# ganslate-team/ganslate

Measured on AMD Instinct MI355X. Metric: training images/sec, CycleGAN ResNet-9 256x256 bf16, higher is better.
Workload: dtype bf16; 1 GPU; horse2zebra CycleGAN ResNet-9 + PatchGAN-3, 256x256, batch 8 per GPU, lsgan, lambda 10/10, pool 50, Adam(2e-4, 0.5), SSIM + D-output metrics on; global_batch=8, parallelism=dp1

## Files before the change

### ganslate_amd/csrc/common.hpp

```cpp
#pragma once
#include <hip/hip_runtime.h>
#include <stdint.h>
#include <type_traits>
#include "../../include/ganslate_hip.h"

typedef __attribute__((ext_vector_type(8))) short bf16x8;
typedef __attribute__((ext_vector_type(4))) short s16x4;
typedef __attribute__((ext_vector_type(4))) float f32x4;
typedef __attribute__((ext_vector_type(2))) float f32x2;
typedef __attribute__((ext_vector_type(2))) __bf16 bf16x2_t;

#define GS_LDS(p) ((__attribute__((address_space(3))) void*)(p))
#define GS_GLB(p) ((const __attribute__((address_space(1))) void*)(p))

__device__ __forceinline__ float bf2f(unsigned short h) { return __uint_as_float(((unsigned)h) << 16); }
__device__ __forceinline__ float bf_lo(unsigned u) { return __uint_as_float(u << 16); }
__device__ __forceinline__ float bf_hi(unsigned u) { return __uint_as_float(u & 0xffff0000u); }
__device__ __forceinline__ unsigned pack_bf2(float a, float b) {
  f32x2 v = {a, b};
  bf16x2_t r = __builtin_convertvector(v, bf16x2_t);
  return *reinterpret_cast<unsigned*>(&r);
}
__device__ __forceinline__ unsigned short f2bf(float a) { return (unsigned short)(pack_bf2(a, 0.f) & 0xffffu); }
__device__ __forceinline__ void unpack_bf8(float* f, const uint4 v) {
  f[0] = bf_lo(v.x); f[1] = bf_hi(v.x); f[2] = bf_lo(v.y); f[3] = bf_hi(v.y);
  f[4] = bf_lo(v.z); f[5] = bf_hi(v.z); f[6] = bf_lo(v.w); f[7] = bf_hi(v.w);
}
__device__ __forceinline__ void add_bf8(float* f, const uint4 v) {
  f[0] += bf_lo(v.x); f[1] += bf_hi(v.x); f[2] += bf_lo(v.y); f[3] += bf_hi(v.y);
  f[4] += bf_lo(v.z); f[5] += bf_hi(v.z); f[6] += bf_lo(v.w); f[7] += bf_hi(v.w);
}
__device__ __forceinline__ uint4 pack_bf8(const float* f) {
  uint4 o;
  o.x = pack_bf2(f[0], f[1]); o.y = pack_bf2(f[2], f[3]); o.z = pack_bf2(f[4], f[5]); o.w = pack_bf2(f[6], f[7]);
  return o;
}

__device__ __forceinline__ void glds16(const void* gsrc, void* lds_wave_base) {
  __builtin_amdgcn_global_load_lds(GS_GLB(gsrc), GS_LDS(lds_wave_base), 16, 0, 0);
}

__device__ __forceinline__ unsigned lds_addr(const void* p) {
  return (unsigned)(size_t)(__attribute__((address_space(3))) const char*)p;
}
template <int OFF>
__device__ __forceinline__ void lds_read128(bf16x8& v, unsigned addr) {
  asm volatile("ds_read_b128 %0, %1 offset:%2" : "=v"(v) : "v"(addr), "i"(OFF) : "memory");
}
template <int N>
__device__ __forceinline__ void gs_lgkm_wait(bf16x8& a, bf16x8& b, bf16x8& c, bf16x8& d, bf16x8& e, bf16x8& f) {
  asm volatile("s_waitcnt lgkmcnt(%6)" : "+v"(a), "+v"(b), "+v"(c), "+v"(d), "+v"(e), "+v"(f) : "i"(N) : "memory");
}
template <int N>
__device__ __forceinline__ void gs_lgkm_wait(bf16x8& a, bf16x8& b, bf16x8& c, bf16x8& d, bf16x8& e) {
  asm volatile("s_waitcnt lgkmcnt(%5)" : "+v"(a), "+v"(b), "+v"(c), "+v"(d), "+v"(e) : "i"(N) : "memory");
}
template <int N>
__device__ __forceinline__ void gs_lgkm_wait(bf16x8& a, bf16x8& b, bf16x8& c, bf16x8& d, bf16x8& e, bf16x8& f,
                                             bf16x8& g, bf16x8& h) {
  asm volatile("s_waitcnt lgkmcnt(%8)"
               : "+v"(a), "+v"(b), "+v"(c), "+v"(d), "+v"(e), "+v"(f), "+v"(g), "+v"(h) : "i"(N) : "memory");
}

template <int N>
__device__ __forceinline__ void gs_lgkm_wait_only() { asm volatile("s_waitcnt lgkmcnt(%0)" ::"i"(N) : "memory"); }
__device__ __forceinline__ void reg_fence(bf16x8& x) { asm volatile("" : "+v"(x)); }

__device__ __forceinline__ void lds_barrier() {
  asm volatile("s_waitcnt lgkmcnt(0)" ::: "memory");
  __builtin_amdgcn_s_barrier();
  asm volatile("" ::: "memory");
}

template <int OFF>
__device__ __forceinline__ void lds_read64_tr(uint2& v, unsigned addr) {
  asm volatile("ds_read_b64_tr_b16 %0, %1 offset:%2" : "=v"(v) : "v"(addr), "i"(OFF) : "memory");
}
template <int N>
__device__ __forceinline__ void gs_lgkm_wait64(uint2& a, uint2& b) {
  asm volatile("s_waitcnt lgkmcnt(%2)" : "+v"(a), "+v"(b) : "i"(N) : "memory");
}
template <int N>
__device__ __forceinline__ void gs_lgkm_wait64(uint2& a, uint2& b, uint2& c, uint2& d, uint2& e, uint2& f) {
  asm volatile("s_waitcnt lgkmcnt(%6)" : "+v"(a), "+v"(b), "+v"(c), "+v"(d), "+v"(e), "+v"(f) : "i"(N) : "memory");
}
template <int B, int E, class F>
__device__ __forceinline__ void static_for(F&& f) {
  if constexpr (B < E) {
    f(std::integral_constant<int, B>{});
    static_for<B + 1, E>(f);
  }
}

__device__ __forceinline__ int div_small(int m, int d, float rcp) {
  int q = (int)((float)m * rcp);
  int r = m - q * d;
  if (r < 0) { --q; } else if (r >= d) { ++q; }
  return q;
}

__device__ __forceinline__ int border_index(int x, int n, int mode, bool& ok) {
  const bool inb = (unsigned)x < (unsigned)n;
  int xr = x < 0 ? -x : x;
  xr = xr >= n ? 2 * n - 2 - xr : xr;
  int xc = x < 0 ? 0 : x;
  xc = xc >= n ? n - 1 : xc;
  ok = ok & (inb | (mode != GS_BORDER_ZERO));
  return mode == GS_BORDER_REFLECT ? xr : (mode == GS_BORDER_REPLICATE ? xc : x);
}

__device__ __forceinline__ float apply_act(float v, int act, float slope) {
  if (act == GS_ACT_RELU) return v > 0.f ? v : 0.f;
  if (act == GS_ACT_LRELU) return v > 0.f ? v : v * slope;
  if (act == GS_ACT_TANH) return tanhf(v);
  return v;
}
static __device__ __noinline__ float gs_tanh_call(float v) { return tanhf(v); }
__device__ __forceinline__ float apply_act_small(float v, int act, float slope) {
  if (act == GS_ACT_RELU) return v > 0.f ? v : 0.f;
  if (act == GS_ACT_LRELU) return v > 0.f ? v : v * slope;
  if (act == GS_ACT_TANH) return gs_tanh_call(v);
  return v;
}
__device__ __forceinline__ float act_grad_from_out(float o, int act, float slope) {
  if (act == GS_ACT_RELU) return o > 0.f ? 1.f : 0.f;
  if (act == GS_ACT_LRELU) return o > 0.f ? 1.f : slope;
  if (act == GS_ACT_TANH) return 1.f - o * o;
  return 1.f;
}

__device__ __forceinline__ float inorm_dy(float g, float yh, float m, float s1, float s2, float rs) {
  const float gh = __fmul_rn(g, m);
  return __fmul_rn(rs, __fsub_rn(__fsub_rn(gh, s1), __fmul_rn(yh, s2)));
}

template <int CTRL>
__device__ __forceinline__ float dpp_mov(float v) {
  return __builtin_bit_cast(float, __builtin_amdgcn_update_dpp(0, __builtin_bit_cast(int, v), CTRL, 0xf, 0xf, false));
}
__device__ __forceinline__ float row16_sum(float v) {
  v += dpp_mov<0xB1>(v);
  v += dpp_mov<0x4E>(v);
  v += dpp_mov<0x141>(v);
  v += dpp_mov<0x140>(v);
  return v;
}
__device__ __forceinline__ float row_sum_stride4(float v) { v += dpp_mov<0x124>(v); v += dpp_mov<0x128>(v); return v; }
__device__ __forceinline__ float row_sum_stride8(float v) { v += dpp_mov<0x128>(v); return v; }

__device__ __forceinline__ float wave_sum(float v) {
#pragma unroll
  for (int o = 32; o > 0; o >>= 1) v += __shfl_xor(v, o, 64);
  return v;
}
template <typename P, int MAX_THREADS>
__global__ __launch_bounds__(MAX_THREADS) void final_sum_kernel(const P* partial, int n, double scale, float* out) {
  __shared__ double sh[256];
  double s = 0.0;
  for (int i = threadIdx.x; i < n; i += 256) s += (double)partial[i];
  sh[threadIdx.x] = s;
  __syncthreads();
  for (int o = 128; o > 0; o >>= 1) {
    if ((int)threadIdx.x < o) sh[threadIdx.x] += sh[threadIdx.x + o];
    __syncthreads();
  }
  if (threadIdx.x == 0) out[0] = (float)(sh[0] * scale);
}

__device__ __forceinline__ void adam_one(float& p, float& g, float& m, float& v, float b1, float b2, float eps,
                                         float bc2_sqrt, float step_size, float gscale, int zero_grad) {
  const float gi = g * gscale;
  const float mi = m + (gi - m) * (1.f - b1);
  const float vi = v * b2 + (1.f - b2) * gi * gi;
  const float denom = sqrtf(vi) / bc2_sqrt + eps;
  p = p - step_size * (mi / denom);
  m = mi;
  v = vi;
  if (zero_grad) g = 0.f;
}


#define GS_OPTIONS(X) \
  X(SPLITK, "splitk", 1)                        \
  X(SPLITK_MAX_BLOCKS, "splitk_max_blocks", 128)  \
  X(SPLITK_TARGET, "splitk_target", 256)        \
  X(HCONV, "hconv", 1)                          \
  X(HCONV_WIDE, "hconv_wide", 1)                \
  X(HWGRAD, "hwgrad", 1)                        \
  X(HWGRAD_WIDE, "hwgrad_wide", 1)              \
  X(HWGRAD_PLANES, "hwgrad_planes", 1)          \
  X(NORM_BWD_PPB, "norm_bwd_ppb", 0)            \
  X(NORM_APPLY_UNROLL, "norm_apply_unroll", 4)  \
  X(GCONV_TILE288, "gconv_tile288", 1)          \
  X(GCONV_MULTI, "gconv_multi", 1)              \
  X(HCONVW_RING, "hconvw_ring", 1)              \
  X(HCONVT, "hconvt", 192)                      \
                                                \
  X(HSTRIP, "hstrip", 1024)                     \
  X(WFOLD_ROWS, "wfold_rows", 1)                \
  X(HWGRAD_FT, "hwgrad_ft", 1)                  \
  X(GCONV_BIG, "gconv_big", 192)                \
  X(HCONV_BOX8, "hconv_box8", 1)                \
  X(HCONVW_PERSIST, "hconvw_persist", 1)        \
  X(HSTRIP_REGS, "hstrip_regs", 1)              \
  X(GCONV_TWIN, "gconv_twin", 1)                \
  X(WGRAD_TWIN, "wgrad_twin", 1)                \
  X(GCONV_PERSIST, "gconv_persist", 16)         \
                                                \
  X(HCONVT_PERSIST, "hconvt_persist", 1)        \
  X(WGRAD_ROWS, "wgrad_rows", 1)                \
  X(SPLITK_MULTI, "splitk_multi", 1)            \
  X(SPLITK_RING, "splitk_ring", 1)              \
  X(GCONV_RING4, "gconv_ring4", 16)             \
  X(HCONV5, "hconv5", 64)                       \
                                                \
  X(HCONV5_SEG, "hconv5_seg", 0)                \
  X(HWGRAD2, "hwgrad2", 2)                      \
                                                \
  X(HCONV2, "hconv2", 4)                        \
                                                \
                                                \
  X(PWISE, "pwise", 8)                          \
  X(DAXIS, "daxis", 8192)                          \
                                                \
enum GsOpt {
#define GS_OPT_ENUM(id, name, def) GS_OPT_##id,
  GS_OPTIONS(GS_OPT_ENUM)
#undef GS_OPT_ENUM
  GS_OPT_COUNT
};
int gs_opt(int id);

void gs_set_error(const char* fmt, ...);
const void* gs_zero_page();
void* gs_dump_page();
#define GS_CHECK_HIP(x)                                                                  \
  do {                                                                                   \
    hipError_t e_ = (x);                                                                 \
    if (e_ != hipSuccess) {                                                              \
      gs_set_error("%s failed: %s (%s:%d)", #x, hipGetErrorString(e_), __FILE__, __LINE__); \
      return 1;                                                                          \
    }                                                                                    \
  } while (0)
#define GS_REQUIRE(cond, ...)      \
  do {                             \
    if (!(cond)) {                 \
      gs_set_error(__VA_ARGS__);   \
      return 2;                    \
    }                              \
  } while (0)
```

### ganslate_amd/csrc/wgrad.hip

```cpp
#include "internal.hpp"
#include <cstdlib>

struct WGradK {
  const char* a;
  const char* g;
  float* dw;
  const char* zero;
  int tiles_p, tiles_q, splits, chunk, q_shift;
  float rcp_wa, rcp_hw, rcp_da;
  float* ws;
  long long ws_stride;
  int nets, splits_net, m_net;
  int vec, rmw;
  long long dw_delta;
  int adam;
  gs_adam_fuse ad;
  gs_wgrad_desc d;
};

__device__ __forceinline__ int wg_swz(int R) { return ((R & 3) << 1) | (((R >> 3) & 1) << 3); }

template <int BP, int BQ, int WP, int WQ, bool VOL = true>
__global__ __launch_bounds__(WP * WQ * 64) void wgrad_kernel(const WGradK p) {
  constexpr int NW = WP * WQ, BK = 64, NSTAGE = 3;
  constexpr int ARB = BP * 2, GRB = BQ * 2;
  constexpr int AT = BK * ARB, GT = BK * GRB, STAGE = AT + GT;
  constexpr int ARI = 1024 / ARB, GRI = 1024 / GRB;
  constexpr int A_INSTR = BK / ARI;
  constexpr int NAI = (A_INSTR + NW - 1) / NW, NGI = BK / GRI / NW;
  constexpr int LOADS = NAI + NGI;
  constexpr int TI = BP / WP / 16, TJ = BQ / WQ / 16;
  constexpr int ASW = ARB / 16 - 1 < 15 ? ARB / 16 - 1 : 15;
  static_assert((BK / GRI) % NW == 0, "gathered tile must split evenly over the waves");
  static_assert(NAI == 1 || (A_INSTR % NW == 0 && (ARI * NW) % 16 == 0), "dense tile DMA layout");
  extern __shared__ __attribute__((aligned(16))) char smem[];
  int* taps = reinterpret_cast<int*>(smem + NSTAGE * STAGE);
  char* dummy = smem + NSTAGE * STAGE + GS_MAX_TAPS * 4;
  const gs_wgrad_desc& d = p.d;
  const int tid = threadIdx.x;
  const int wave = __builtin_amdgcn_readfirstlane(tid >> 6);
  const int lane = tid & 63;

  int b = blockIdx.x;
  const int tq = b % p.tiles_q;
  b /= p.tiles_q;
  const int tp = b % p.tiles_p;
  b /= p.tiles_p;
  const int sp = b;
  const int HW = d.Ha * d.Wa;
  const int net = p.nets > 1 ? sp / p.splits_net : 0;
  const int k0 = net * p.m_net + (sp - net * p.splits_net) * p.chunk;
  const int k1 = min((net + 1) * p.m_net, k0 + p.chunk);
  if (k0 >= k1) return;

  for (int t = tid; t < d.T; t += NW * 64)
    taps[t] = ((int)d.dh[t] & 0xff) | (((int)d.dw_[t] & 0xff) << 8) | ((int)d.dd[t] << 16);
  __syncthreads();

  const char* a_n = p.a + (size_t)d.a_co * 2;
  const char* g_n = p.g + (size_t)d.g_co * 2;
  const unsigned g_img = (unsigned)(d.Dg * d.Hg * d.Wg);
  const int a_row0 = ARI * wave + lane / (ARB / 16);
  const int a_slot = lane % (ARB / 16);
  const int a_chunk = a_slot ^ (wg_swz(a_row0) & ASW);
  const int a_pch = tp * BP + a_chunk * 8;
  const bool a_cv = a_pch < d.P;
  const int g_row0 = GRI * wave + lane / (GRB / 16);
  const int g_slot = lane % (GRB / 16);
  const int g_chunk = g_slot ^ wg_swz(g_row0);
  const int g_col = tq * BQ + g_chunk * 8;
  const int g_t = (g_col >> 3) >> p.q_shift;
  const int g_q8 = (g_col >> 3) & ((1 << p.q_shift) - 1);
  const bool g_tv = g_t < d.T;
  const int tpv = taps[g_tv ? g_t : 0];
  const int g_dh = (int)(signed char)(tpv & 0xff), g_dw = (int)(signed char)((tpv >> 8) & 0xff), g_dd = tpv >> 16;
  static_assert((GRI * NW) % 16 == 0, "row step must keep the swizzle invariant");

  int gn[NGI], gz[NGI], gi[NGI], gj[NGI];
#pragma unroll
  for (int i = 0; i < NGI; ++i) {
    const int m = k0 + g_row0 + i * GRI * NW;
    const int nz = div_small(m, HW, p.rcp_hw);
    const int rem = m - nz * HW;
    gi[i] = div_small(rem, d.Wa, p.rcp_wa);
    gj[i] = rem - gi[i] * d.Wa;
    gn[i] = VOL ? div_small(nz, d.Da, p.rcp_da) : nz;
    gz[i] = VOL ? nz - gn[i] * d.Da : 0;
  }

  auto issue = [&](int ks, int buf) {
    char* sb = smem + buf * STAGE;
    const int mb = k0 + ks * BK;
#pragma unroll
    for (int i = 0; i < NAI; ++i) {
      const int R = a_row0 + i * ARI * NW;
      const int m = mb + R;
      unsigned off = ((unsigned)m * (unsigned)d.a_cs + (unsigned)a_pch) * 2u;
      asm volatile("" : "+v"(off));
      const bool real = A_INSTR % NW == 0 || wave + i * NW < A_INSTR;
      const char* src = (real && m < k1 && a_cv) ? a_n + off : p.zero;
      glds16(src, real ? sb + (wave + i * NW) * 1024 : dummy);
    }
#pragma unroll
    for (int i = 0; i < NGI; ++i) {
      const int R = g_row0 + i * GRI * NW;
      const int m = mb + R;
      bool ok = g_tv && m < k1;
      const int nn = gn[i], zz = gz[i], ii = gi[i], jj = gj[i];
      gj[i] += BK;
      while (gj[i] >= d.Wa) { gj[i] -= d.Wa; ++gi[i]; }
      int iz = 0;
      if constexpr (VOL) {
        while (gi[i] >= d.Ha) { gi[i] -= d.Ha; ++gz[i]; }
        while (gz[i] >= d.Da) { gz[i] -= d.Da; ++gn[i]; }
        iz = border_index(zz * d.si + g_dd, d.Dg, d.border, ok);
      } else {
        while (gi[i] >= d.Ha) { gi[i] -= d.Ha; ++gn[i]; }
      }
      const int ih = border_index(ii * d.si + g_dh, d.Hg, d.border, ok);
      const int iw = border_index(jj * d.si + g_dw, d.Wg, d.border, ok);
      unsigned off = (((unsigned)nn * g_img + (unsigned)((iz * d.Hg + ih) * d.Wg + iw)) * (unsigned)d.g_cs + (unsigned)(g_q8 * 8)) * 2u;
      asm volatile("" : "+v"(off));
      const char* src = ok ? g_n + off : p.zero;
      glds16(src, sb + AT + (wave + i * NW) * 1024);
    }
  };

  f32x4 acc[TI][TJ];
#pragma unroll
  for (int i = 0; i < TI; ++i)
#pragma unroll
    for (int j = 0; j < TJ; ++j) acc[i][j] = f32x4{0.f, 0.f, 0.f, 0.f};

  const int wp = wave / WQ, wq = wave % WQ;
  const int nk = (k1 - k0 + BK - 1) / BK;
  const int fk = lane >> 4;
  const int frr = (lane & 15) >> 2;
  const int fcc = lane & 3;

  int aoff[TI], goff[TJ];
  {
    const int sw = wg_swz(fk * 8 + frr);
    const int sub = (fcc & 1) * 8;
#pragma unroll
    for (int i = 0; i < TI; ++i) {
      const int ch = (wp * (BP / WP) / 8) + i * 2 + (fcc >> 1);
      aoff[i] = (fk * 8 + frr) * ARB + sub + ((ch ^ (sw & ASW)) << 4);
    }
#pragma unroll
    for (int j = 0; j < TJ; ++j) {
      const int ch = (wq * (BQ / WQ) / 8) + j * 2 + (fcc >> 1);
      goff[j] = (fk * 8 + frr) * GRB + sub + ((ch ^ sw) << 4);
    }
  }

  issue(0, 0);
  if (nk > 1) issue(1, 1);

  int cur = 0, nxt2 = 2;
  for (int ks = 0; ks < nk; ++ks) {
    if (ks + 1 < nk) asm volatile("s_waitcnt vmcnt(%0)" ::"n"(LOADS) : "memory");
    else asm volatile("s_waitcnt vmcnt(0)" ::: "memory");
    __builtin_amdgcn_s_barrier();
    if (ks + 2 < nk) issue(ks + 2, nxt2);
    const char* ab = smem + cur * STAGE;
    const char* gb = ab + AT;
#pragma unroll
    for (int kk = 0; kk < 2; ++kk) {
      uint2 ah[TI][2], gh[TJ][2];
#pragma unroll
      for (int h = 0; h < 2; ++h) {
#pragma unroll
        for (int i = 0; i < TI; ++i)
          ah[i][h] = __builtin_bit_cast(uint2, __builtin_amdgcn_ds_read_tr16_b64_v4i16(
              (__attribute__((address_space(3))) s16x4*)GS_LDS(ab + aoff[i] + (kk * 32 + h * 4) * ARB)));
#pragma unroll
        for (int j = 0; j < TJ; ++j)
          gh[j][h] = __builtin_bit_cast(uint2, __builtin_amdgcn_ds_read_tr16_b64_v4i16(
              (__attribute__((address_space(3))) s16x4*)GS_LDS(gb + goff[j] + (kk * 32 + h * 4) * GRB)));
      }
#pragma unroll
      for (int i = 0; i < TI; ++i)
#pragma unroll
        for (int j = 0; j < TJ; ++j)
          acc[i][j] = __builtin_amdgcn_mfma_f32_16x16x32_bf16(
              __builtin_bit_cast(bf16x8, uint4{ah[i][0].x, ah[i][0].y, ah[i][1].x, ah[i][1].y}),
              __builtin_bit_cast(bf16x8, uint4{gh[j][0].x, gh[j][0].y, gh[j][1].x, gh[j][1].y}), acc[i][j], 0, 0, 0);
    }
    cur = cur == 2 ? 0 : cur + 1;
    nxt2 = nxt2 == 2 ? 0 : nxt2 + 1;
  }

  const int frow = lane & 15;
  const int TQ = d.T * d.Q;
  float* const obase = p.ws ? p.ws + (size_t)sp * p.ws_stride : p.dw + (size_t)net * p.dw_delta;
  if (p.vec && (p.ws || p.rmw)) {
    constexpr int CP = BQ + 4;
    static_assert(BP * CP * 4 <= NSTAGE * STAGE, "the output tile must fit the stage buffers");
    static_assert(BQ % 4 == 0 && BQ / 4 <= 64 && 64 % (BQ / 4) == 0, "row = a whole number of 16-byte lanes");
    float* ct = reinterpret_cast<float*>(smem);
    __syncthreads();
#pragma unroll
    for (int i = 0; i < TI; ++i)
#pragma unroll
      for (int r = 0; r < 4; ++r)
#pragma unroll
        for (int j = 0; j < TJ; ++j)
          ct[(wp * (BP / WP) + i * 16 + fk * 4 + r) * CP + wq * (BQ / WQ) + j * 16 + frow] = acc[i][j][r];
    __syncthreads();
    constexpr int LPR = BQ / 4, RPI = 64 / LPR;
    constexpr int NR = (BP + NW * RPI - 1) / (NW * RPI);
    const int c4 = (lane % LPR) * 4, rsub = lane / LPR;
    const int col = tq * BQ + c4;
    const bool rmw = p.ws == nullptr && !d.dw_fresh;
    f32x4 old[NR];
#pragma unroll
    for (int it = 0; it < NR; ++it) {
      const int rr = (it * NW + wave) * RPI + rsub, pp = tp * BP + rr;
      old[it] = f32x4{0.f, 0.f, 0.f, 0.f};
      if (rmw && rr < BP && pp < d.P && col < TQ) old[it] = *reinterpret_cast<const f32x4*>(obase + (size_t)pp * d.dw_ld + col);
    }
#pragma unroll
    for (int it = 0; it < NR; ++it) {
      const int rr = (it * NW + wave) * RPI + rsub, pp = tp * BP + rr;
      if (rr < BP && pp < d.P && col < TQ) {
        const f32x4 v = *reinterpret_cast<const f32x4*>(ct + rr * CP + c4);
        if (p.adam) {
          const size_t e = (size_t)pp * d.dw_ld + col;
          const float b1 = p.ad.hyper[1], b2 = p.ad.hyper[2], eps = p.ad.hyper[3], bc2_sqrt = p.ad.hyper[5];
          const float step_size = p.ad.hyper[0] / p.ad.hyper[4];
          float4 P = *reinterpret_cast<const float4*>(p.ad.p + e), M = *reinterpret_cast<const float4*>(p.ad.m + e);
          float4 V = *reinterpret_cast<const float4*>(p.ad.v + e), G = {v[0], v[1], v[2], v[3]};
          adam_one(P.x, G.x, M.x, V.x, b1, b2, eps, bc2_sqrt, step_size, 1.0f, 0);
          adam_one(P.y, G.y, M.y, V.y, b1, b2, eps, bc2_sqrt, step_size, 1.0f, 0);
          adam_one(P.z, G.z, M.z, V.z, b1, b2, eps, bc2_sqrt, step_size, 1.0f, 0);
          adam_one(P.w, G.w, M.w, V.w, b1, b2, eps, bc2_sqrt, step_size, 1.0f, 0);
          *reinterpret_cast<float4*>(p.ad.p + e) = P;
          *reinterpret_cast<float4*>(p.ad.m + e) = M;
          *reinterpret_cast<float4*>(p.ad.v + e) = V;
          const uint2 o = {pack_bf2(P.x, P.y), pack_bf2(P.z, P.w)};
          const size_t grp = e >> 3, half = (e >> 2) & 1;
          const int jf = p.ad.inv_f ? p.ad.inv_f[grp] : -1, jd = p.ad.inv_d ? p.ad.inv_d[grp] : -1;
          if (jf >= 0) static_cast<uint2*>(p.ad.fpack)[(size_t)jf * 2 + half] = o;
          if (jd >= 0) static_cast<uint2*>(p.ad.dpack)[(size_t)jd * 2 + half] = o;
          if (p.ad.tr_pack) *reinterpret_cast<float4*>(ct + rr * CP + c4) = P;
        } else {
          *reinterpret_cast<f32x4*>(obase + (size_t)pp * d.dw_ld + col) = old[it] + v;
        }
      }
    }
    if (p.adam && p.ad.tr_pack) {
      __syncthreads();
      constexpr int RG = BP / 8;
      for (int gi = threadIdx.x; gi < RG * BQ; gi += NW * 64) {
        int rg, cc;
        if constexpr (RG % 4 == 0 && BQ % 16 == 0) {
          cc = ((gi >> 6) % (BQ / 16)) * 16 + (gi & 15);
          rg = (gi / (64 * (BQ / 16))) * 4 + ((gi >> 4) & 3);
        } else {
          rg = gi / BQ; cc = gi - rg * BQ;
        }
        const int colt = tq * BQ + cc, p0 = tp * BP + rg * 8;
        if (colt < TQ && p0 < d.P) {
          const int t = colt >> (3 + p.q_shift), q = colt & ((8 << p.q_shift) - 1);
          const int base = p.ad.tr_base[t];
          if (base >= 0) {
            float f[8];
#pragma unroll
            for (int k8 = 0; k8 < 8; ++k8) f[k8] = ct[(rg * 8 + k8) * CP + cc];
            const uint4 o = {pack_bf2(f[0], f[1]), pack_bf2(f[2], f[3]), pack_bf2(f[4], f[5]), pack_bf2(f[6], f[7])};
            *reinterpret_cast<uint4*>(static_cast<char*>(p.ad.tr_pack) +
                                      ((size_t)base + (size_t)q * p.ad.tr_kp[t] + p0) * 2) = o;
          }
        }
      }
    }
    return;
  }
#pragma unroll
  for (int i = 0; i < TI; ++i) {
#pragma unroll
    for (int r = 0; r < 4; ++r) {
      const int pp = tp * BP + wp * (BP / WP) + i * 16 + fk * 4 + r;
      if (pp < d.P) {
        float* row = obase + (size_t)pp * d.dw_ld;
#pragma unroll
        for (int j = 0; j < TJ; ++j) {
          const int col = tq * BQ + wq * (BQ / WQ) + j * 16 + frow;
          if (col < TQ) {
            if (p.ws) row[col] = acc[i][j][r];
            else unsafeAtomicAdd(row + col, acc[i][j][r]);
          }
        }
      }
    }
  }
}

namespace {
template <int BP, int BQ, int WP, int WQ, bool VOL = true>
int launch_wgrad_impl(WGradK& k, const gs_wgrad_desc* d, hipStream_t st, int plan_only, int* slabs) {
  k.tiles_p = (d->P + BP - 1) / BP;
  k.tiles_q = (d->T * d->Q + BQ - 1) / BQ;
  const long long M = (long long)d->N / k.nets * d->Da * d->Ha * d->Wa;
  GS_REQUIRE(M * k.nets < (1 << 24) && M * k.nets * d->a_cs < (1LL << 31) &&
                 (long long)d->N * d->Dg * d->Hg * d->Wg * d->g_cs < (1LL << 31),
             "gs_wgrad: tensor too large for 32-bit offsets");
  const long long tiles = (long long)k.tiles_p * k.tiles_q * k.nets;
  const long long max_splits = (M + 1023) / 1024 > 0 ? (M + 1023) / 1024 : 1;
  long long splits = 1;
  double best = 1e30;
  for (int r = 1; r <= 4; ++r) {
    long long s = (256LL * r) / tiles;
    if (s < 1) s = 1;
    if (s > max_splits) s = max_splits;
    const long long blocks = tiles * s;
    const long long rounds = (blocks + 255) / 256;
    const double cost = (double)rounds * ((double)M / (double)s + 512.0);
    if (cost < best) { best = cost; splits = s; }
  }
  int chunk = (int)((M + splits - 1) / splits);
  chunk = (chunk + 63) / 64 * 64;
  splits = (M + chunk - 1) / chunk;
  k.splits = (int)splits * k.nets;
  k.splits_net = (int)splits;
  k.m_net = (int)M;
  k.chunk = chunk;
  k.rcp_hw = 1.0f / (float)(d->Ha * d->Wa);
  const long long blocks = tiles * splits;
  GS_REQUIRE(blocks > 0 && blocks < (1LL << 31), "gs_wgrad: bad grid %lld", blocks);
  *slabs = splits == 1 ? 0 : (int)splits;
  if (splits == 1) k.ws = nullptr;
  k.rmw = splits == 1 && gs_opt(GS_OPT_WGRAD_ROWS) != 0;
  k.vec = gs_opt(GS_OPT_WGRAD_ROWS) != 0 && (reinterpret_cast<uintptr_t>(k.dw) & 15) == 0 && (k.dw_delta & 3) == 0 &&
          (reinterpret_cast<uintptr_t>(k.ws) & 15) == 0 && (k.ws_stride & 3) == 0;
  if (plan_only) return 0;
  GS_REQUIRE(!k.adam || (splits == 1 && k.vec && k.rmw && k.nets == 1 && d->dw_ld % 8 == 0),
             "gs_wgrad_adam: not a one-split launch with 16-byte rows (gs_wgrad_adam_eligible)");
  constexpr int lds = 3 * 64 * (BP + BQ) * 2 + GS_MAX_TAPS * 4 + 1024;
  if (int rc = gs_allow_lds<&wgrad_kernel<BP, BQ, WP, WQ, VOL>>(lds)) return rc;
  hipLaunchKernelGGL((wgrad_kernel<BP, BQ, WP, WQ, VOL>), dim3((unsigned)blocks), dim3(WP * WQ * 64), lds, st, k);
  GS_CHECK_HIP(hipGetLastError());
  return 0;
}
template <int BP, int BQ, int WP, int WQ>
int launch_wgrad(WGradK& k, const gs_wgrad_desc* d, hipStream_t st, int plan_only, int* slabs) {
  if (d->Da == 1 && d->Dg == 1) return launch_wgrad_impl<BP, BQ, WP, WQ, false>(k, d, st, plan_only, slabs);
  return launch_wgrad_impl<BP, BQ, WP, WQ, true>(k, d, st, plan_only, slabs);
}
}

template <int EL>
__global__ __launch_bounds__(256) void wgrad_reduce_kernel(const float4* ws, float4* dw, long long n4, int slabs,
                                                           long long stride4, long long ws_y4, long long dw_y4) {
  ws += (long long)blockIdx.y * ws_y4;
  dw += (long long)blockIdx.y * dw_y4;
  constexpr int SL = 256 / EL;
  __shared__ float4 part[SL][EL];
  const int el = threadIdx.x % EL, sl = threadIdx.x / EL;
  for (long long e0 = (long long)blockIdx.x * EL; e0 < n4; e0 += (long long)gridDim.x * EL) {
    const long long e = e0 + el;
    float4 s = {0.f, 0.f, 0.f, 0.f};
    if (e < n4) {
      int k = sl;
      for (; k + 3 * SL < slabs; k += 4 * SL) {
        float4 t[4];
#pragma unroll
        for (int u = 0; u < 4; ++u) t[u] = ws[(long long)(k + u * SL) * stride4 + e];
#pragma unroll
        for (int u = 0; u < 4; ++u) { s.x += t[u].x; s.y += t[u].y; s.z += t[u].z; s.w += t[u].w; }
      }
      for (; k < slabs; k += SL) {
        const float4 t = ws[(long long)k * stride4 + e];
        s.x += t.x; s.y += t.y; s.z += t.z; s.w += t.w;
      }
    }
    part[sl][el] = s;
    __syncthreads();
    if (sl == 0 && e < n4) {
      float4 o = dw[e];
#pragma unroll 4
      for (int l = 0; l < SL; ++l) { o.x += part[l][el].x; o.y += part[l][el].y; o.z += part[l][el].z; o.w += part[l][el].w; }
      dw[e] = o;
    }
    __syncthreads();
  }
}
static inline void launch_slab_reduce(const float* ws, float* dst, long long n4, int slabs, long long stride4,
                                      hipStream_t st, int nets = 1, long long ws_y4 = 0, long long dw_y4 = 0) {
  const float4* w4 = reinterpret_cast<const float4*>(ws);
  float4* d4 = reinterpret_cast<float4*>(dst);
  const unsigned ny = (unsigned)nets;
  if (n4 <= 4 && slabs > 16)
    hipLaunchKernelGGL(wgrad_reduce_kernel<4>, dim3(1, ny), dim3(256), 0, st, w4, d4, n4, slabs, stride4, ws_y4, dw_y4);
  else if (n4 <= 16 && slabs > 16)
    hipLaunchKernelGGL(wgrad_reduce_kernel<16>, dim3(1, ny), dim3(256), 0, st, w4, d4, n4, slabs, stride4, ws_y4, dw_y4);
  else {
    long long blocks = (n4 + 63) / 64;
    if (blocks > 4096) blocks = 4096;
    hipLaunchKernelGGL(wgrad_reduce_kernel<64>, dim3((unsigned)blocks, ny), dim3(256), 0, st, w4, d4, n4, slabs, stride4, ws_y4,
                       dw_y4);
  }
}

void gs_launch_slab_reduce(const float* ws, float* dst, long long n4, int slabs, long long stride4, hipStream_t st, int nets,
                           long long ws_y4, long long dw_y4) {
  launch_slab_reduce(ws, dst, n4, slabs, stride4, st, nets, ws_y4, dw_y4);
}

namespace {
int wgrad_generic(const gs_wgrad_desc* d, const void* a, const void* g, float* dw, float* ws, int plan_only,
                  void* stream, int* slabs, const gs_twin* tw = nullptr, const gs_adam_fuse* adam = nullptr) {
  WGradK k;
  k.nets = tw ? 2 : 1;
  k.dw_delta = tw ? tw->dw_delta / 4 : 0;
  k.a = static_cast<const char*>(a);
  k.g = static_cast<const char*>(g);
  k.dw = dw;
  k.ws = ws;
  k.ws_stride = (long long)d->P * d->dw_ld;
  k.adam = adam ? 1 : 0;
  if (adam) k.ad = *adam; else k.ad = gs_adam_fuse{};
  k.zero = static_cast<const char*>(gs_zero_page());
  GS_REQUIRE(k.zero || plan_only, "gs_wgrad: library not initialised (call gs_init)");
  int sh = 0;
  while ((8 << sh) < d->Q) ++sh;
  k.q_shift = sh;
  k.rcp_wa = 1.0f / (float)d->Wa;
  k.rcp_da = 1.0f / (float)d->Da;
  k.d = *d;
  hipStream_t st = static_cast<hipStream_t>(stream);
  if (d->P <= 16) return launch_wgrad<16, 256, 1, 8>(k, d, st, plan_only, slabs);
  if (d->P <= 64) return launch_wgrad<64, 256, 1, 8>(k, d, st, plan_only, slabs);
  return launch_wgrad<128, 256, 4, 4>(k, d, st, plan_only, slabs);
}

int wgrad_check(const gs_wgrad_desc* d) {
  GS_REQUIRE(d->Q >= 8 && (d->Q & 7) == 0 && ((d->Q >> 3) & ((d->Q >> 3) - 1)) == 0,
             "gs_wgrad: Q=%d must be 8*2^k", d->Q);
  GS_REQUIRE((d->P & 7) == 0, "gs_wgrad: P=%d must be a multiple of 8", d->P);
  GS_REQUIRE(d->T >= 1 && d->T <= GS_MAX_TAPS, "gs_wgrad: T=%d out of range", d->T);
  GS_REQUIRE((d->a_cs & 7) == 0 && (d->a_co & 7) == 0 && (d->g_cs & 7) == 0 && (d->g_co & 7) == 0,
             "gs_wgrad: channel strides/offsets must be multiples of 8");
  GS_REQUIRE(d->Da >= 1 && d->Dg >= 1, "gs_wgrad: depths must be >= 1 (1 for 2-D tensors)");
  GS_REQUIRE(d->dw_ld == d->T * d->Q, "gs_wgrad: dw_ld must be T * Q");
  return 0;
}

int reduce_slabs(const float* ws, float* dw, int slabs, long long slab, const gs_twin* tw, void* stream) {
  hipStream_t st = static_cast<hipStream_t>(stream);
  if (tw && tw->dw_delta % 16 == 0 && ((size_t)slabs * slab) % 4 == 0) {
    launch_slab_reduce(ws, dw, slab / 4, slabs, slab / 4, st, 2, (long long)slabs * slab / 4, tw->dw_delta / 16);
  } else {
    launch_slab_reduce(ws, dw, slab / 4, slabs, slab / 4, st);
    if (tw) launch_slab_reduce(ws + (size_t)slabs * slab, dw + tw->dw_delta / 4, slab / 4, slabs, slab / 4, st);
  }
  GS_CHECK_HIP(hipGetLastError());
  return 0;
}

int wgrad_impl(const gs_wgrad_desc* d, const void* a1, const void* g1, const void* a2, const void* g2, float* dw,
               float* ws, int64_t ws_floats, int plan_only, void* stream, int64_t* need_floats, const gs_twin* tw = nullptr) {
  if (int rc = wgrad_check(d)) return rc;
  const long long slab = (long long)d->P * d->dw_ld;
  const bool det = ws != nullptr || plan_only;
  int handled = 0;
  if (!a2 && !tw)
    if (int rc = gs_pwise_wgrad_try(d, a1, g1, dw, det ? ws : nullptr, plan_only, stream, &handled)) return rc;
  if (!handled)
    if (int rc = gs_hwgrad_try2(d, a1, g1, a2, g2, dw, det ? ws : nullptr, plan_only, stream, &handled, tw)) return rc;
  if (handled) {
    const int nets = tw ? 2 : 1;
    if (need_floats) *need_floats = (int64_t)nets * handled * slab;
    if (plan_only || !det) return 0;
    GS_REQUIRE(ws_floats >= (int64_t)nets * handled * slab, "gs_wgrad_ws: workspace of %lld floats, %lld needed",
               (long long)ws_floats, (long long)nets * handled * slab);
    return reduce_slabs(ws, dw, handled, slab, tw, stream);
  }
  if (tw) {
    gs_wgrad_desc half = *d;
    half.N = d->N / 2;
    int hh = 0;
    static const char dummy = 0;
    if (int rc = gs_hwgrad_try2(&half, &dummy, &dummy, a2 ? &dummy : nullptr, a2 ? &dummy : nullptr, nullptr, nullptr, 1, nullptr,
                                &hh, nullptr)) return rc;
    if (hh || !gs_opt(GS_OPT_WGRAD_TWIN)) {
      if (need_floats) *need_floats = -1;
      GS_REQUIRE(plan_only, "gs_wgrad_ws_twin: this layer's kernel has no twin form (gs_wgrad_twin_native): run the two halves");
      return 0;
    }
  }
  const int nets = tw ? 2 : 1;
  int64_t need = 0;
  gs_wgrad_desc second = *d;
  second.dw_fresh = 0;
  for (int pass = 0; pass < (a2 ? 2 : 1); ++pass) {
    int slabs = 0;
    if (int rc = wgrad_generic(pass ? &second : d, pass ? a2 : a1, pass ? g2 : g1, dw, det ? ws : nullptr, plan_only, stream,
                               &slabs, tw))
      return rc;
    if ((int64_t)nets * slabs * slab > need) need = (int64_t)nets * slabs * slab;
    if (plan_only || !det) continue;
    GS_REQUIRE(ws_floats >= (int64_t)nets * slabs * slab, "gs_wgrad_ws: workspace of %lld floats, %lld needed",
               (long long)ws_floats, (long long)nets * slabs * slab);
    if (slabs > 0)
      if (int rc = reduce_slabs(ws, dw, slabs, slab, tw, stream)) return rc;
  }
  if (need_floats) *need_floats = need;
  return 0;
}

int64_t wgrad_probe(const gs_wgrad_desc* d, int pair, bool twin) {
  static const char dummy = 0;
  const void* second = pair ? &dummy : nullptr;
  gs_twin t{};
  t.n_split = d->N / 2;
  int64_t need = 0;
  return wgrad_impl(d, &dummy, &dummy, second, second, nullptr, nullptr, 0, 1, nullptr, &need, twin ? &t : nullptr) ? -1 : need;
}
}

extern "C" int gs_wgrad(const gs_wgrad_desc* d, const void* a, const void* g, float* dw, void* stream) {
  GS_REQUIRE(d && a && g && dw, "gs_wgrad: null argument");
  return wgrad_impl(d, a, g, nullptr, nullptr, dw, nullptr, 0, 0, stream, nullptr);
}

extern "C" int gs_wgrad_adam_eligible(const gs_wgrad_desc* d) {
  if (!d || wgrad_check(d) || !gs_opt(GS_OPT_WGRAD_ROWS) || d->dw_ld % 8) return 0;
  static const char dummy = 0;
  int handled = 0;
  if (gs_pwise_wgrad_try(d, &dummy, &dummy, nullptr, nullptr, 1, nullptr, &handled) || handled) return 0;
  if (gs_hwgrad_try2(d, &dummy, &dummy, nullptr, nullptr, nullptr, nullptr, 1, nullptr, &handled, nullptr) || handled) return 0;
  int slabs = -1;
  if (wgrad_generic(d, &dummy, &dummy, nullptr, nullptr, 1, nullptr, &slabs) || slabs != 0) return 0;
  return 1;
}
extern "C" int gs_wgrad_adam(const gs_wgrad_desc* d, const void* a, const void* g, const gs_adam_fuse* adam, void* stream) {
  GS_REQUIRE(d && a && g && adam && adam->p && adam->m && adam->v && adam->hyper, "gs_wgrad_adam: null argument");
  GS_REQUIRE((adam->inv_f == nullptr) == (adam->fpack == nullptr) && (adam->inv_d == nullptr) == (adam->dpack == nullptr),
             "gs_wgrad_adam: an index table and its pack go together");
  GS_REQUIRE(((reinterpret_cast<uintptr_t>(adam->p) | reinterpret_cast<uintptr_t>(adam->m) | reinterpret_cast<uintptr_t>(adam->v) |
               reinterpret_cast<uintptr_t>(adam->fpack) | reinterpret_cast<uintptr_t>(adam->dpack)) & 15) == 0,
             "gs_wgrad_adam: buffers must be 16-byte aligned");
  GS_REQUIRE((adam->tr_pack == nullptr) == (adam->tr_base == nullptr) && (adam->tr_pack == nullptr) == (adam->tr_kp == nullptr) &&
                 (reinterpret_cast<uintptr_t>(adam->tr_pack) & 15) == 0,
             "gs_wgrad_adam: the transposed pack comes with both of its tables, 16-byte aligned");
  GS_REQUIRE(gs_wgrad_adam_eligible(d), "gs_wgrad_adam: this layer does not run as a one-split im2col launch (gs_wgrad_adam_eligible)");
  gs_wgrad_desc fresh = *d;
  fresh.dw_fresh = 1;
  int slabs = 0;
  return wgrad_generic(&fresh, a, g, adam->p, nullptr, 0, stream, &slabs, nullptr, adam);
}

extern "C" int gs_wgrad_pair(const gs_wgrad_desc* d, const void* a1, const void* g1, const void* a2, const void* g2,
                             float* dw, void* stream) {
  GS_REQUIRE(d && a1 && g1 && a2 && g2 && dw, "gs_wgrad_pair: null argument");
  return wgrad_impl(d, a1, g1, a2, g2, dw, nullptr, 0, 0, stream, nullptr);
}

extern "C" int64_t gs_wgrad_ws_floats(const gs_wgrad_desc* d, int32_t pair) {
  return d ? wgrad_probe(d, pair, false) : 0;
}
extern "C" int gs_wgrad_ws(const gs_wgrad_desc* d, const void* a1, const void* g1, const void* a2, const void* g2,
                           float* dw, float* ws, int64_t ws_floats, void* stream) {
  GS_REQUIRE(d && a1 && g1 && dw && (a2 == nullptr) == (g2 == nullptr), "gs_wgrad_ws: null argument");
  GS_REQUIRE(ws || gs_wgrad_ws_floats(d, a2 != nullptr) == 0, "gs_wgrad_ws: this layer needs a workspace (gs_wgrad_ws_floats)");
  return wgrad_impl(d, a1, g1, a2, g2, dw, ws, ws_floats, 0, stream, nullptr);
}

extern "C" int gs_wgrad_twin_native(const gs_wgrad_desc* d, int32_t pair) {
  if (!d || d->N < 2 || (d->N & 1)) return 0;
  return wgrad_probe(d, pair, true) >= 0;
}
extern "C" int64_t gs_wgrad_ws_floats_twin(const gs_wgrad_desc* d, int32_t pair) {
  return d ? wgrad_probe(d, pair, true) : -1;
}
extern "C" int gs_wgrad_ws_twin(const gs_wgrad_desc* d, const void* a1, const void* g1, const void* a2, const void* g2,
                                float* dw, float* ws, int64_t ws_floats, const gs_twin* tw, void* stream) {
  GS_REQUIRE(d && a1 && g1 && dw && ws && tw && (a2 == nullptr) == (g2 == nullptr), "gs_wgrad_ws_twin: null argument");
  GS_REQUIRE(2 * tw->n_split == d->N, "gs_wgrad_ws_twin: the two networks take the same number of images");
  return wgrad_impl(d, a1, g1, a2, g2, dw, ws, ws_floats, 0, stream, nullptr, tw);
}

template <int COLS>
__global__ __launch_bounds__(256) void bias_grad_kernel(const unsigned short* dy, long long pixels, int C8, int cs,
                                                        int co, float* db, int pix_per_block, float* ws) {
  constexpr int ROWS = 256 / COLS;
  __shared__ float red[ROWS][COLS][9];
  const int tid = threadIdx.x;
  const int col = tid % COLS, row = tid / COLS;
  const int c8 = blockIdx.y * COLS + col;
  const long long p0 = (long long)blockIdx.x * pix_per_block;
  const long long p1 = min(pixels, p0 + pix_per_block);
  float a[8];
#pragma unroll
  for (int k = 0; k < 8; ++k) a[k] = 0.f;
  if (c8 < C8)
    for (long long px = p0 + row; px < p1; px += ROWS) {
      const uint4 v = *reinterpret_cast<const uint4*>(dy + px * cs + co + c8 * 8);
      a[0] += bf_lo(v.x); a[1] += bf_hi(v.x); a[2] += bf_lo(v.y); a[3] += bf_hi(v.y);
      a[4] += bf_lo(v.z); a[5] += bf_hi(v.z); a[6] += bf_lo(v.w); a[7] += bf_hi(v.w);
    }
#pragma unroll
  for (int k = 0; k < 8; ++k) red[row][col][k] = a[k];
  __syncthreads();
  for (int o = tid; o < COLS * 8; o += 256) {
    const int cc = o >> 3, k = o & 7;
    const int ch8 = blockIdx.y * COLS + cc;
    if (ch8 < C8) {
      float s = 0.f;
#pragma unroll
      for (int r = 0; r < ROWS; ++r) s += red[r][cc][k];
      if (ws) ws[(size_t)blockIdx.x * C8 * 8 + ch8 * 8 + k] = s;
      else unsafeAtomicAdd(db + ch8 * 8 + k, s);
    }
  }
}

__global__ __launch_bounds__(256) void bias_head_reduce_kernel(const float* __restrict__ ws, float* db, int slabs, int C,
                                                               int c_valid) {
  __shared__ float part[32][8];
  const int c = threadIdx.x & 7, sl = threadIdx.x >> 3;
  float s = 0.f;
  int k = sl;
  for (; k + 96 < slabs; k += 128) {
    float t[4];
#pragma unroll
    for (int u = 0; u < 4; ++u) t[u] = ws[(size_t)(k + 32 * u) * C + c];
#pragma unroll
    for (int u = 0; u < 4; ++u) s += t[u];
  }
  for (; k < slabs; k += 32) s += ws[(size_t)k * C + c];
  part[sl][c] = s;
  __syncthreads();
  if (threadIdx.x < c_valid) {
    float o = db[threadIdx.x];
#pragma unroll 4
    for (int l = 0; l < 32; ++l) o += part[l][threadIdx.x];
    db[threadIdx.x] = o;
  }
}

static int bias_grad_impl(const void* dy, int64_t pixels, int32_t C, int32_t cs, int32_t co, float* db, float* ws,
                          int64_t ws_floats, int plan_only, void* stream, int64_t* need, int c_valid = -1) {
  GS_REQUIRE(pixels > 0 && C > 0 && (C & 7) == 0 && (cs & 7) == 0 && (co & 7) == 0,
             "gs_bias_grad: bad argument (C, cs, co must be multiples of 8)");
  const int C8 = C / 8;
  int ppb = (int)((pixels + 1023) / 1024);
  if (ppb < 64) ppb = 64;
  const unsigned bx = (unsigned)((pixels + ppb - 1) / ppb);
  if (need) *need = (int64_t)bx * C;
  if (plan_only) return 0;
  GS_REQUIRE(dy && db, "gs_bias_grad: null argument");
  GS_REQUIRE(!ws || ws_floats >= (int64_t)bx * C, "gs_bias_grad_ws: workspace too small");
  hipStream_t st = static_cast<hipStream_t>(stream);
  const unsigned short* p = static_cast<const unsigned short*>(dy);
  if (C8 >= 32) hipLaunchKernelGGL((bias_grad_kernel<32>), dim3(bx, (C8 + 31) / 32), dim3(256), 0, st, p, (long long)pixels, C8, cs, co, db, ppb, ws);
  else if (C8 >= 8) hipLaunchKernelGGL((bias_grad_kernel<8>), dim3(bx, (C8 + 7) / 8), dim3(256), 0, st, p, (long long)pixels, C8, cs, co, db, ppb, ws);
  else if (C8 >= 2) hipLaunchKernelGGL((bias_grad_kernel<2>), dim3(bx, (C8 + 1) / 2), dim3(256), 0, st, p, (long long)pixels, C8, cs, co, db, ppb, ws);
  else hipLaunchKernelGGL((bias_grad_kernel<1>), dim3(bx, C8), dim3(256), 0, st, p, (long long)pixels, C8, cs, co, db, ppb, ws);
  GS_CHECK_HIP(hipGetLastError());
  if (ws && c_valid >= 0) {
    hipLaunchKernelGGL(bias_head_reduce_kernel, dim3(1), dim3(256), 0, st, ws, db, (int)bx, C, c_valid);
    GS_CHECK_HIP(hipGetLastError());
  } else if (ws) {
    const long long n4 = C / 4;
    launch_slab_reduce(ws, db, n4, (int)bx, n4, st);
    GS_CHECK_HIP(hipGetLastError());
  }
  return 0;
}

extern "C" int gs_bias_grad(const void* dy, int64_t pixels, int32_t C, int32_t cs, int32_t co, float* db,
                            void* stream) {
  return bias_grad_impl(dy, pixels, C, cs, co, db, nullptr, 0, 0, stream, nullptr);
}
extern "C" int64_t gs_bias_grad_ws_floats(int64_t pixels, int32_t C) {
  int64_t need = 0;
  return bias_grad_impl(nullptr, pixels, C, 8, 0, nullptr, nullptr, 0, 1, nullptr, &need) ? -1 : need;
}
extern "C" int gs_bias_grad_ws(const void* dy, int64_t pixels, int32_t C, int32_t cs, int32_t co, float* db, float* ws,
                               int64_t ws_floats, void* stream) {
  GS_REQUIRE(ws, "gs_bias_grad_ws: null workspace");
  return bias_grad_impl(dy, pixels, C, cs, co, db, ws, ws_floats, 0, stream, nullptr);
}
extern "C" int gs_bias_grad_head_ws(const void* dy, int64_t pixels, int32_t cs, int32_t co, int32_t c_valid, float* db,
                                    float* ws, int64_t ws_floats, void* stream) {
  GS_REQUIRE(ws && c_valid > 0 && c_valid <= 8, "gs_bias_grad_head_ws: null workspace or c_valid outside 1..8");
  return bias_grad_impl(dy, pixels, 8, cs, co, db, ws, ws_floats, 0, stream, nullptr, c_valid);
}
```

Measured before the change: 494.2 img/s.

## Pipeline LDS fragment reads with MFMAs, remap blocks per XCD, strength-reduce gather addressing

The wgrad kernel's inner loop is restructured so LDS transpose reads for both k-halves are issued up front and interleaved with MFMAs using explicit lgkmcnt waits and register fences, overlapping LDS latency with matrix math. Block indices are remapped so consecutive tiles land on the same XCD, improving L2 locality. Gather and dense address computation is strength-reduced: offsets are incremented per stage instead of recomputed, wrap loops become single conditional carries, and 24-bit multiplies are used. A new guard enforces the 24-bit range and assumes BK never wraps a dimension more than once.

New measurement: 503.0 img/s, median of 6. 1.8% higher.

```diff
diff --git a/ganslate_amd/csrc/common.hpp b/ganslate_amd/csrc/common.hpp
--- a/ganslate_amd/csrc/common.hpp
+++ b/ganslate_amd/csrc/common.hpp
@@ -84,6 +84,7 @@
 __device__ __forceinline__ void gs_lgkm_wait64(uint2& a, uint2& b, uint2& c, uint2& d, uint2& e, uint2& f) {
   asm volatile("s_waitcnt lgkmcnt(%6)" : "+v"(a), "+v"(b), "+v"(c), "+v"(d), "+v"(e), "+v"(f) : "i"(N) : "memory");
 }
+__device__ __forceinline__ void reg_fence(uint2& lo, uint2& hi) { asm volatile("" : "+v"(lo), "+v"(hi)); }
 template <int B, int E, class F>
 __device__ __forceinline__ void static_for(F&& f) {
   if constexpr (B < E) {
diff --git a/ganslate_amd/csrc/wgrad.hip b/ganslate_amd/csrc/wgrad.hip
--- a/ganslate_amd/csrc/wgrad.hip
+++ b/ganslate_amd/csrc/wgrad.hip
@@ -41,7 +41,8 @@
   const int wave = __builtin_amdgcn_readfirstlane(tid >> 6);
   const int lane = tid & 63;
 
-  int b = blockIdx.x;
+  const int nblk = (int)gridDim.x, xper = nblk >> 3, xrem = nblk & 7, xcd = (int)blockIdx.x & 7;
+  int b = (xcd < xrem ? xcd * (xper + 1) : xrem * (xper + 1) + (xcd - xrem) * xper) + ((int)blockIdx.x >> 3);
   const int tq = b % p.tiles_q;
   b /= p.tiles_q;
   const int tp = b % p.tiles_p;
@@ -76,7 +77,8 @@
   const int g_dh = (int)(signed char)(tpv & 0xff), g_dw = (int)(signed char)((tpv >> 8) & 0xff), g_dd = tpv >> 16;
   static_assert((GRI * NW) % 16 == 0, "row step must keep the swizzle invariant");
 
-  int gn[NGI], gz[NGI], gi[NGI], gj[NGI];
+  int gz[NGI], gi[NGI], gj[NGI];
+  unsigned gnb[NGI];
 #pragma unroll
   for (int i = 0; i < NGI; ++i) {
     const int m = k0 + g_row0 + i * GRI * NW;
@@ -84,9 +86,19 @@
     const int rem = m - nz * HW;
     gi[i] = div_small(rem, d.Wa, p.rcp_wa);
     gj[i] = rem - gi[i] * d.Wa;
-    gn[i] = VOL ? div_small(nz, d.Da, p.rcp_da) : nz;
-    gz[i] = VOL ? nz - gn[i] * d.Da : 0;
-  }
+    const int n = VOL ? div_small(nz, d.Da, p.rcp_da) : nz;
+    gz[i] = VOL ? nz - n * d.Da : 0;
+    gnb[i] = (unsigned)n * g_img;
+  }
+  const int s_nz = div_small(BK, HW, p.rcp_hw), s_rem = BK - s_nz * HW;
+  const int s_i = div_small(s_rem, d.Wa, p.rcp_wa), s_j = s_rem - s_i * d.Wa;
+  const int s_n = VOL ? div_small(s_nz, d.Da, p.rcp_da) : s_nz, s_z = VOL ? s_nz - s_n * d.Da : 0;
+  const unsigned s_nb = (unsigned)s_n * g_img;
+  unsigned a_off[NAI];
+#pragma unroll
+  for (int i = 0; i < NAI; ++i)
+    a_off[i] = ((unsigned)(k0 + a_row0 + i * ARI * NW) * (unsigned)d.a_cs + (unsigned)a_pch) * 2u;
+  const unsigned a_step = (unsigned)BK * (unsigned)d.a_cs * 2u;
 
   auto issue = [&](int ks, int buf) {
     char* sb = smem + buf * STAGE;
@@ -95,7 +107,8 @@
     for (int i = 0; i < NAI; ++i) {
       const int R = a_row0 + i * ARI * NW;
       const int m = mb + R;
-      unsigned off = ((unsigned)m * (unsigned)d.a_cs + (unsigned)a_pch) * 2u;
+      unsigned off = a_off[i];
+      a_off[i] += a_step;
       asm volatile("" : "+v"(off));
       const bool real = A_INSTR % NW == 0 || wave + i * NW < A_INSTR;
       const char* src = (real && m < k1 && a_cv) ? a_n + off : p.zero;
@@ -106,20 +119,29 @@
       const int R = g_row0 + i * GRI * NW;
       const int m = mb + R;
       bool ok = g_tv && m < k1;
-      const int nn = gn[i], zz = gz[i], ii = gi[i], jj = gj[i];
-      gj[i] += BK;
-      while (gj[i] >= d.Wa) { gj[i] -= d.Wa; ++gi[i]; }
-      int iz = 0;
+      const int zz = gz[i], ii = gi[i], jj = gj[i];
+      const unsigned nb = gnb[i];
+      gj[i] += s_j;
+      int c = gj[i] >= d.Wa;
+      gj[i] -= c ? d.Wa : 0;
+      gi[i] += s_i + c;
+      c = gi[i] >= d.Ha;
+      gi[i] -= c ? d.Ha : 0;
+      unsigned lin;
       if constexpr (VOL) {
-        while (gi[i] >= d.Ha) { gi[i] -= d.Ha; ++gz[i]; }
-        while (gz[i] >= d.Da) { gz[i] -= d.Da; ++gn[i]; }
-        iz = border_index(zz * d.si + g_dd, d.Dg, d.border, ok);
+        gz[i] += s_z + c;
+        c = gz[i] >= d.Da;
+        gz[i] -= c ? d.Da : 0;
+        const int iz = border_index((int)__umul24(zz, d.si) + g_dd, d.Dg, d.border, ok);
+        const int ih = border_index((int)__umul24(ii, d.si) + g_dh, d.Hg, d.border, ok);
+        lin = (unsigned)(((int)__umul24(iz, d.Hg) + ih) * d.Wg);
       } else {
-        while (gi[i] >= d.Ha) { gi[i] -= d.Ha; ++gn[i]; }
+        const int ih = border_index((int)__umul24(ii, d.si) + g_dh, d.Hg, d.border, ok);
+        lin = __umul24(ih, d.Wg);
       }
-      const int ih = border_index(ii * d.si + g_dh, d.Hg, d.border, ok);
-      const int iw = border_index(jj * d.si + g_dw, d.Wg, d.border, ok);
-      unsigned off = (((unsigned)nn * g_img + (unsigned)((iz * d.Hg + ih) * d.Wg + iw)) * (unsigned)d.g_cs + (unsigned)(g_q8 * 8)) * 2u;
+      gnb[i] += s_nb + (c ? g_img : 0u);
+      const int iw = border_index((int)__umul24(jj, d.si) + g_dw, d.Wg, d.border, ok);
+      unsigned off = ((nb + lin + (unsigned)iw) * (unsigned)d.g_cs + (unsigned)(g_q8 * 8)) * 2u;
       asm volatile("" : "+v"(off));
       const char* src = ok ? g_n + off : p.zero;
       glds16(src, sb + AT + (wave + i * NW) * 1024);
@@ -162,31 +184,42 @@
     if (ks + 1 < nk) asm volatile("s_waitcnt vmcnt(%0)" ::"n"(LOADS) : "memory");
     else asm volatile("s_waitcnt vmcnt(0)" ::: "memory");
     __builtin_amdgcn_s_barrier();
+    constexpr int NF = TI + TJ;
+    const unsigned ab = lds_addr(smem) + (unsigned)(cur * STAGE), gb = ab + AT;
+    uint2 fr[2][NF][2];
+    auto rd = [&](auto kf) {
+      constexpr int kk = decltype(kf)::value / NF, f = decltype(kf)::value % NF;
+      if constexpr (f == 0 || f > TJ) {
+        constexpr int i = f == 0 ? 0 : f - TJ;
+        lds_read64_tr<kk * 32 * ARB>(fr[kk][f][0], ab + (unsigned)aoff[i]);
+        lds_read64_tr<(kk * 32 + 4) * ARB>(fr[kk][f][1], ab + (unsigned)aoff[i]);
+      } else {
+        constexpr int j = f - 1;
+        lds_read64_tr<kk * 32 * GRB>(fr[kk][f][0], gb + (unsigned)goff[j]);
+        lds_read64_tr<(kk * 32 + 4) * GRB>(fr[kk][f][1], gb + (unsigned)goff[j]);
+      }
+    };
     if (ks + 2 < nk) issue(ks + 2, nxt2);
-    const char* ab = smem + cur * STAGE;
-    const char* gb = ab + AT;
-#pragma unroll
-    for (int kk = 0; kk < 2; ++kk) {
-      uint2 ah[TI][2], gh[TJ][2];
-#pragma unroll
-      for (int h = 0; h < 2; ++h) {
-#pragma unroll
-        for (int i = 0; i < TI; ++i)
-          ah[i][h] = __builtin_bit_cast(uint2, __builtin_amdgcn_ds_read_tr16_b64_v4i16(
-              (__attribute__((address_space(3))) s16x4*)GS_LDS(ab + aoff[i] + (kk * 32 + h * 4) * ARB)));
-#pragma unroll
-        for (int j = 0; j < TJ; ++j)
-          gh[j][h] = __builtin_bit_cast(uint2, __builtin_amdgcn_ds_read_tr16_b64_v4i16(
-              (__attribute__((address_space(3))) s16x4*)GS_LDS(gb + goff[j] + (kk * 32 + h * 4) * GRB)));
+    static_for<0, NF>(rd);
+    static_for<0, 2 * TI * TJ>([&](auto mm) {
+      constexpr int kk = decltype(mm)::value / (TI * TJ), i = decltype(mm)::value % (TI * TJ) / TJ, j = decltype(mm)::value % TJ;
+      constexpr int F = i == 0 ? j + 1 : (j == 0 ? TJ + i : 0);
+      if constexpr (F > 0) {
+        constexpr int ahead = kk == 1 ? 0 : (F == 1 ? 0 : F);
+        __builtin_amdgcn_sched_barrier(0);
+        gs_lgkm_wait_only<2 * (NF - 1 - F) + 2 * ahead>();
+        if constexpr (F == 1) reg_fence(fr[kk][0][0], fr[kk][0][1]);
+        reg_fence(fr[kk][F][0], fr[kk][F][1]);
+        if constexpr (kk == 0) {
+          if constexpr (F == 1) rd(std::integral_constant<int, NF>{});
+          rd(std::integral_constant<int, NF + F>{});
+        }
       }
-#pragma unroll
-      for (int i = 0; i < TI; ++i)
-#pragma unroll
-        for (int j = 0; j < TJ; ++j)
-          acc[i][j] = __builtin_amdgcn_mfma_f32_16x16x32_bf16(
-              __builtin_bit_cast(bf16x8, uint4{ah[i][0].x, ah[i][0].y, ah[i][1].x, ah[i][1].y}),
-              __builtin_bit_cast(bf16x8, uint4{gh[j][0].x, gh[j][0].y, gh[j][1].x, gh[j][1].y}), acc[i][j], 0, 0, 0);
-    }
+      constexpr int fa = i == 0 ? 0 : TJ + i, fg = 1 + j;
+      acc[i][j] = __builtin_amdgcn_mfma_f32_16x16x32_bf16(
+          __builtin_bit_cast(bf16x8, uint4{fr[kk][fa][0].x, fr[kk][fa][0].y, fr[kk][fa][1].x, fr[kk][fa][1].y}),
+          __builtin_bit_cast(bf16x8, uint4{fr[kk][fg][0].x, fr[kk][fg][0].y, fr[kk][fg][1].x, fr[kk][fg][1].y}), acc[i][j], 0, 0, 0);
+    });
     cur = cur == 2 ? 0 : cur + 1;
     nxt2 = nxt2 == 2 ? 0 : nxt2 + 1;
   }
@@ -306,6 +339,8 @@
   GS_REQUIRE(M * k.nets < (1 << 24) && M * k.nets * d->a_cs < (1LL << 31) &&
                  (long long)d->N * d->Dg * d->Hg * d->Wg * d->g_cs < (1LL << 31),
              "gs_wgrad: tensor too large for 32-bit offsets");
+  GS_REQUIRE(d->si >= 1 && d->si < (1 << 24) && d->Dg < (1 << 24) && d->Hg < (1 << 24) && d->Wg < (1 << 24),
+             "gs_wgrad: stride or gathered extent outside the 24-bit coordinate arithmetic of the kernel");
   const long long tiles = (long long)k.tiles_p * k.tiles_q * k.nets;
   const long long max_splits = (M + 1023) / 1024 > 0 ? (M + 1023) / 1024 : 1;
   long long splits = 1;
```
